# DeepLearnPhysics/u-resnet

Measured on AMD Instinct MI355X. Metric: fwd+bwd images/sec on 3D 192^3x1 U-ResNet, higher is better.
Workload: dtype f32

## Files before the change

### u-resnet_amd/csrc/conv_api.hip

```cpp
#include <dlfcn.h>
#include <stdarg.h>
#include <stdlib.h>
#include <stdio.h>
#include <string.h>

#include "bf16_common.h"

static thread_local char g_err[1024] = "";
void ursn_set_error(const char* fmt, ...) {
  va_list ap;
  va_start(ap, fmt);
  vsnprintf(g_err, sizeof(g_err), fmt, ap);
  va_end(ap);
}
extern "C" const char* ursn_last_error(void) { return g_err; }
static thread_local const char* g_kernel = "";
static long g_kernel_launches = 0;
void ursn_note_kernel(const char* name) { g_kernel = name; ++g_kernel_launches; }
void ursn_relabel_kernel(const char* name) { g_kernel = name; }
long ursn_kernel_launch_count() { return g_kernel_launches; }
extern "C" const char* ursn_last_kernel_name() { return g_kernel; }
extern "C" int ursn_abi_version(void) { return URSN_ABI_VERSION; }

namespace {
// ... 192 lines not shown
              ++nt;
            }
        g.ntaps = nt;
      }
  return ncls;
}

int conv_dispatch(const ursn_conv_desc& d, ConvPass pass, const float* in, const float* w, float* out, int accumulate,
                  hipStream_t s);

static int run_gather(const ursn_conv_desc& d, ConvPass pass, const float* in, const float* w, float* out,
                      int accumulate, hipStream_t s) {
  GatherGeom g[8];
  int n = build_geoms(d, pass, g);
  if (n < 0) return 2;
  for (int i = 0; i < n; ++i) {
    g[i].accumulate = accumulate;
    if (g[i].ntaps == 0 && accumulate) continue;
    if (d.algo == 1) URSN_TRY(launch_gconv_naive(g[i], in, w, out, s));
    else URSN_TRY(launch_gconv_mfma(g[i], in, w, out, s));
  }
  return 0;
}

int tiled_conv_supported(const ursn_conv_desc& d, ConvPass pass);
int launch_tiled_conv(const ursn_conv_desc& d, ConvPass pass, const float* in, const float* w, float* out,
                      int accumulate, hipStream_t s);

static float* op_scratch_floats(size_t n) {
  static float* buf = nullptr;
  static size_t cap = 0;
  if (n > cap) {
    if (buf) (void)hipFree(buf);
    buf = nullptr; cap = 0;
    if (hipMalloc((void**)&buf, n * sizeof(float)) != hipSuccess) return nullptr;
    cap = n;
  }
  return buf;
}

int conv_dispatch(const ursn_conv_desc& d, ConvPass pass, const float* in, const float* w, float* out, int accumulate,
                  hipStream_t s) {
  if (d.vdz_z) {
    URSN_REQUIRE(pass == PASS_DGRAD && d.vdz_coef && d.vdz_out && tiled_conv_supported(d, pass), "conv: BatchNorm-backward apply on load (vdz_z) not supported for this shape / pass");
    return launch_tiled_conv(d, pass, in, w, out, accumulate, s);
  }
  if (d.bs_partial) {
    URSN_REQUIRE(pass == PASS_DGRAD && tiled_conv_supported(d, pass), "conv: fused BatchNorm-backward reductions (bs_partial) not supported for this shape / pass");
    return launch_tiled_conv(d, pass, in, w, out, accumulate, s);
  }
  if (d.in_mean && pass != PASS_DGRAD) {
    URSN_REQUIRE(d.in_rstd && d.in_beta && tiled_conv_supported(d, pass), "conv: normalise-on-load (in_mean) not supported for this shape / pass");
    return launch_tiled_conv(d, pass, in, w, out, accumulate, s);
  }
  if (d.pw_dy) {
    URSN_REQUIRE(pass == PASS_DGRAD, "conv: fused pointwise term (pw_dy) applies to the data gradient only");
    if (tiled_deconv_supported(d, pass))
      return launch_tiled_deconv(d, pass, in, w, out, accumulate, nullptr, 0.f, nullptr, nullptr, s);
    if (!d.in_split && igemm_conv_supported(d, pass))
      return launch_igemm_conv(d, pass, in, w, out, accumulate, nullptr, 0.f, nullptr, nullptr, s);
    URSN_REQUIRE(tiled_conv_supported(d, pass), "conv: fused pointwise term (pw_dy) not supported for this shape");
    return launch_tiled_conv(d, pass, in, w, out, accumulate, s);
  }
  if (d.in_split) {
    if (pointwise_conv_supported(d, pass, accumulate))
      return launch_pointwise_conv(d, pass, in, w, out, accumulate, nullptr, 0.f, nullptr, nullptr, s);
    URSN_REQUIRE(tiled_conv_supported(d, pass), "conv: split input (in_split=%d) not supported for this shape", d.in_split);
    return launch_tiled_conv(d, pass, in, w, out, accumulate, s);
  }
  if (d.algo == 3) {
    if (tiled_deconv_supported(d, pass))
      return launch_tiled_deconv(d, pass, in, w, out, accumulate, nullptr, 0.f, nullptr, nullptr, s);
    URSN_REQUIRE(tiled_conv_supported(d, pass), "tiled conv kernel does not support this shape");
    return launch_tiled_conv(d, pass, in, w, out, accumulate, s);
  }
  if (d.algo == 4) {
    URSN_REQUIRE(igemm_conv_supported(d, pass), "igemm conv kernel does not support this shape");
    return launch_igemm_conv(d, pass, in, w, out, accumulate, nullptr, 0.f, nullptr, nullptr, s);
  }
  if (d.algo == 7) {
    URSN_REQUIRE(lds_scatter_supported(d, pass), "LDS scatter conv kernel does not support this shape");
    return launch_lds_scatter(d, pass, in, w, out, accumulate, nullptr, 0.f, nullptr, nullptr, s);
  }
  if (d.algo == 6) {
    URSN_REQUIRE(stride2_conv_supported(d, pass), "stride-2 conv kernel does not support this shape");
    return launch_stride2_conv(d, pass, in, w, out, accumulate, nullptr, 0.f, nullptr, nullptr, s);
  }
  if ((d.algo == 0 || d.algo == 5) && pointwise_conv_supported(d, pass, accumulate))
    return launch_pointwise_conv(d, pass, in, w, out, accumulate, nullptr, 0.f, nullptr, nullptr, s);
  URSN_REQUIRE(d.algo != 5, "pointwise conv kernel does not support this shape");
  if (d.algo == 0 && deep_conv_supported(d, pass)) {
    float* sc = op_scratch_floats(deep_conv_scratch_floats(d, pass));
    URSN_REQUIRE(sc, "conv: no memory for the deep-level kernel's packed weights");
    return launch_deep_conv(d, pass, in, w, out, accumulate, sc, nullptr, 0.f, nullptr, nullptr, s);
  }
  if (d.algo == 0 && igemm_conv_supported(d, pass))
    return launch_igemm_conv(d, pass, in, w, out, accumulate, nullptr, 0.f, nullptr, nullptr, s);
  if (d.algo == 0 && tiled_conv_supported(d, pass)) return launch_tiled_conv(d, pass, in, w, out, accumulate, s);
  if (d.algo == 0 && prefer_lds_scatter(d, pass))
    return launch_lds_scatter(d, pass, in, w, out, accumulate, nullptr, 0.f, nullptr, nullptr, s);
  if (d.algo == 0 && tiled_deconv_supported(d, pass))
    return launch_tiled_deconv(d, pass, in, w, out, accumulate, nullptr, 0.f, nullptr, nullptr, s);
  if (d.algo == 0 && stride2_conv_supported(d, pass))
    return launch_stride2_conv(d, pass, in, w, out, accumulate, nullptr, 0.f, nullptr, nullptr, s);
  return run_gather(d, pass, in, w, out, accumulate, s);
}

static bf16_t* op_wpack(size_t elems) {
  static bf16_t* buf = nullptr;
  static size_t cap = 0;
  if (elems > cap) {
    if (buf) (void)hipFree(buf);
    buf = nullptr; cap = 0;
    if (hipMalloc((void**)&buf, elems * sizeof(bf16_t)) != hipSuccess) return nullptr;
    cap = elems;
  }
  return buf;
}
static void stored_weight_strides(GatherGeom& g, int Kr, int Nr) { g.w_tap_stride = Kr * Nr; g.w_sk = Nr; g.w_sn = 1; }

static int bf16_conv_op(const ursn_conv_desc& d0, ConvPass pass, const void* in, const float* w, void* out, int accumulate,
                        double* stats_partial, size_t stats_bytes, float eps, float* mean, float* rstd, hipStream_t s) {
  ursn_conv_desc d = d0;
  const bool scalar_in = d.cin == 1;
  if (scalar_in) {
    URSN_REQUIRE(pass == PASS_FWD && !d.transposed && d.k == 3 && d.stride == 1 && !d.in_mean && !d.in_split,
                 "bf16 conv: the scalar fp32 input form (cin = 1) is the k3 s1 forward pass / weight gradient only");
    d.cin = 8; d.in_cstride = 8;
  }
  if (d.in_split) {
    URSN_REQUIRE(pass == PASS_DGRAD && d.in_split == 8 && d.cin == 16 && d.dx2 && d.pw_dy,
                 "bf16 conv: a split tensor is supported as the two-tensor output (dx, dx2) of the 16 -> 8 data gradient with the fused shortcut term");
    if (d.in_cstride <= 0) d.in_cstride = 8;
  }
  GatherGeom g[8];
  const int n = build_geoms(d, pass, g);
  URSN_REQUIRE(n >= 1, "bf16 conv: bad descriptor");
  int64_t V = (int64_t)d.n;
  for (int j = 0; j < 3; ++j) V *= g[0].out_d[j];
  URSN_REQUIRE(!stats_partial || n == 1 || pass == PASS_FWD, "bf16 conv: statistics only on forward passes");
  if (d.pw_dy && n == 1 && !b3conv_ok(g[0]) && bcbconv_pw_ok(g[0])) {
    URSN_REQUIRE(pass == PASS_DGRAD && d.pw_w && !d.in_split && !d.in_mean && !stats_partial, "bf16 conv: the fused shortcut term belongs to a plain data gradient");
    bf16_t* wp = op_wpack(bcbconv_pack_elems(g[0]));
    URSN_REQUIRE(wp, "bf16 conv: no memory for the packed weights");
    g[0].accumulate = accumulate;
    return launch_bcbconv(g[0], (const bf16_t*)in, w, 0, 0, wp, (bf16_t*)out, nullptr, s, (const bf16_t*)d.pw_dy,
                          d.pw_dy_cstride > 0 ? d.pw_dy_cstride : d.cout, d.pw_w);
  }
  if (scalar_in || d.in_mean || d.pw_dy) {
    URSN_REQUIRE(n == 1 && b3conv_ok(g[0]), "bf16 conv: fused forms (cin = 1 / in_mean / pw_dy) need a 3-D k3 s1 layer with 8 / 16 channels");
    bf16_t* wp = op_wpack(b3conv_pack_elems());
    URSN_REQUIRE(wp, "bf16 conv: no memory for the packed weights");
    g[0].accumulate = accumulate;
    const int blocks = bconv_grid_blocks(g[0]);
    URSN_REQUIRE(!stats_partial || bconv_stats_scratch_doubles(g[0]) * sizeof(double) <= stats_bytes, "bf16 conv: statistics scratch too small");
    if (scalar_in && (stored_weight_strides(g[0], 1, d.cout), b0conv_ok(g[0])) && !accumulate) {
      bf16_t* wp0 = op_wpack(b0conv_pack_elems());
      URSN_REQUIRE(wp0, "bf16 conv: no memory for the packed weights");
      const int blocks0 = b0conv_grid_blocks(g[0]);
      URSN_REQUIRE(!stats_partial || (size_t)blocks0 * 32 * sizeof(double) <= stats_bytes, "bf16 conv: statistics scratch too small");
      URSN_TRY(launch_b0conv(g[0], (const float*)in, w, d.cout, wp0, (bf16_t*)out, stats_partial, s));
      if (stats_partial) URSN_TRY(launch_bn_stats_final(stats_partial, blocks0, g[0].Nn, 16, V, eps, mean, rstd, s));
      return 0;
    }
    if (scalar_in) {
      URSN_REQUIRE(g[0].K == 8, "bf16 conv: the scalar input form needs the 8-channel kernel view");
      stored_weight_strides(g[0], 1, d.cout);
// ... 18 lines not shown
  bool empty = false;
  for (int i = 0; i < n; ++i) empty = empty || g[i].ntaps == 0;
  if (empty && !accumulate) {
    URSN_REQUIRE(g[0].out_cs == g[0].Nn, "bf16 conv: overwrite with empty parity classes needs a compact output tensor");
    int64_t e = (int64_t)d.n * g[0].Nn;
    for (int j = 0; j < 3; ++j) e *= g[0].out_d[j];
    URSN_HIP(hipMemsetAsync(out, 0, (size_t)e * sizeof(bf16_t), s));
  }
  if (!stats_partial && bdeconv_ok(g, n)) {
    bf16_t* wp = op_wpack(bdeconv_pack_elems());
    URSN_REQUIRE(wp, "bf16 conv: no memory for the packed weights");
    return launch_bdeconv(g, n, (const bf16_t*)in, w, 0, 0, wp, (bf16_t*)out, nullptr, accumulate, s);
  }
  if (n == 1 && bs2k8_ok(g[0])) {
    bf16_t* wp = op_wpack(bs2k8_pack_elems());
    URSN_REQUIRE(wp, "bf16 conv: no memory for the packed weights");
    const int blocks = bs2k8_grid_blocks(g[0]);
    URSN_REQUIRE(!stats_partial || (size_t)blocks * 32 * sizeof(double) <= stats_bytes, "bf16 conv: statistics scratch too small");
    URSN_TRY(launch_bs2k8(g[0], (const bf16_t*)in, w, 0, 0, wp, (bf16_t*)out, stats_partial, accumulate, nullptr, nullptr, 0, s));
    if (stats_partial) URSN_TRY(launch_bn_stats_final(stats_partial, blocks, g[0].Nn, 16, V, eps, mean, rstd, s));
    return 0;
  }
  if (bsconv_ok(g, n)) {
    bf16_t* wp = op_wpack(bsconv_pack_elems(g, n));
    URSN_REQUIRE(wp, "bf16 conv: no memory for the packed weights");
    URSN_REQUIRE(!stats_partial || bsconv_stats_scratch_doubles(g, n) * sizeof(double) <= stats_bytes, "bf16 conv: statistics scratch too small");
    URSN_TRY(launch_bsconv(g, n, (const bf16_t*)in, w, 0, 0, wp, (bf16_t*)out, stats_partial, accumulate, s));
    if (stats_partial) URSN_TRY(bsconv_stats_finalize(g, n, stats_partial, V, eps, mean, rstd, s));
    return 0;
  }
  for (int i = 0; i < n; ++i) {
    g[i].accumulate = accumulate;
    if (g[i].ntaps == 0) continue;
    bf16_t* wp = op_wpack(bconv_pack_elems(g[i]));
    URSN_REQUIRE(wp, "bf16 conv: unsupported geometry or no memory for the packed weights");
    URSN_REQUIRE(!stats_partial || bconv_stats_scratch_doubles(g[i]) * sizeof(double) * n <= stats_bytes, "bf16 conv: statistics scratch too small");
    URSN_TRY(launch_bconv(g[i], (const bf16_t*)in, w, 0, 0, wp, (bf16_t*)out, (stats_partial && n == 1) ? stats_partial : nullptr, 0, 0, s));
    if (stats_partial && n == 1) URSN_TRY(bconv_stats_finalize(g[i], stats_partial, bconv_grid_blocks(g[i]), V, eps, mean, rstd, s));
  }
  return 0;
}

extern "C" int ursn_conv_forward(const ursn_conv_desc* d, const float* x, const float* w, float* y, void* stream) {
  URSN_REQUIRE(d && x && w && y, "conv_forward: null argument");
  if (d->dtype == 1) return bf16_conv_op(*d, PASS_FWD, x, w, y, 0, nullptr, 0, 0.f, nullptr, nullptr, (hipStream_t)stream);
  return conv_dispatch(*d, PASS_FWD, x, w, y, 0, (hipStream_t)stream);
}

extern "C" int ursn_conv_forward_stats(const ursn_conv_desc* d, const float* x, const float* w, float* y, float* mean,
                                       float* rstd, float eps, void* scratch, size_t scratch_bytes, void* stream) {
  URSN_REQUIRE(d && x && w && y && mean && rstd && scratch, "conv_forward_stats: null argument");
  hipStream_t s = (hipStream_t)stream;
  if (d->dtype == 1) {
    URSN_REQUIRE(!d->transposed, "conv_forward_stats: bf16 transposed convs take their statistics at net level");
    return bf16_conv_op(*d, PASS_FWD, x, w, y, 0, (double*)scratch, scratch_bytes, eps, mean, rstd, s);
  }
  GatherGeom g[8];
  URSN_REQUIRE(build_geoms(*d, PASS_FWD, g) >= 1, "conv_forward_stats: bad descriptor");
  int64_t V = (int64_t)d->n;
  for (int j = 0; j < 3; ++j) V *= g[0].out_d[j];
  if (d->transposed) { V = (int64_t)d->n; for (int j = 0; j < d->ndim; ++j) V *= 2 * d->in_sp[j]; }
  const int ocs = d->out_cstride > 0 ? d->out_cstride : d->cout;
  if (d->in_mean)
    URSN_REQUIRE(d->in_rstd && d->in_beta && tiled_conv_supported(*d, PASS_FWD), "conv_forward_stats: normalise-on-load (in_mean) not supported for this shape");
  if (d->in_split)
    URSN_REQUIRE(pointwise_conv_supported(*d, PASS_FWD, 0) || tiled_conv_supported(*d, PASS_FWD),
                 "conv_forward_stats: split input (in_split=%d) not supported for this shape", d->in_split);
  if ((d->algo == 0 || d->algo == 5 || d->in_split) && pointwise_conv_supported(*d, PASS_FWD, 0)) {
    URSN_REQUIRE(pointwise_stats_scratch_doubles(*d) * sizeof(double) <= scratch_bytes,
                 "conv_forward_stats: scratch too small");
    return launch_pointwise_conv(*d, PASS_FWD, x, w, y, 0, (double*)scratch, eps, mean, rstd, s);
  }
  if (d->algo == 0 && deep_conv_supported(*d, PASS_FWD)) {
    URSN_REQUIRE(deep_conv_stats_scratch_doubles(*d) * sizeof(double) <= scratch_bytes, "conv_forward_stats: scratch too small");
    float* sc = op_scratch_floats(deep_conv_scratch_floats(*d, PASS_FWD));
    URSN_REQUIRE(sc, "conv_forward_stats: no memory for the deep-level kernel's packed weights");
    return launch_deep_conv(*d, PASS_FWD, x, w, y, 0, sc, (double*)scratch, eps, mean, rstd, s);
  }
  if ((d->algo == 0 || d->algo == 4) && igemm_conv_supported(*d, PASS_FWD)) {
    URSN_REQUIRE(igemm_stats_scratch_doubles(*d) * sizeof(double) <= scratch_bytes,
                 "conv_forward_stats: scratch too small");
    return launch_igemm_conv(*d, PASS_FWD, x, w, y, 0, (double*)scratch, eps, mean, rstd, s);
  }
  if ((d->algo == 0 || d->algo == 6) && stride2_conv_supported(*d, PASS_FWD)) {
    URSN_REQUIRE(stride2_stats_scratch_doubles(*d) * sizeof(double) <= scratch_bytes,
                 "conv_forward_stats: scratch too small");
    return launch_stride2_conv(*d, PASS_FWD, x, w, y, 0, (double*)scratch, eps, mean, rstd, s);
  }
  if ((d->algo == 0 && prefer_lds_scatter(*d, PASS_FWD)) || (d->algo == 7 && lds_scatter_supported(*d, PASS_FWD))) {
    URSN_REQUIRE(lds_scatter_stats_scratch_doubles(*d) * sizeof(double) <= scratch_bytes,
                 "conv_forward_stats: scratch too small");
    return launch_lds_scatter(*d, PASS_FWD, x, w, y, 0, (double*)scratch, eps, mean, rstd, s);
  }
  if ((d->algo == 0 || d->algo == 3) && tiled_deconv_supported(*d, PASS_FWD)) {
    URSN_REQUIRE(tiled_deconv_stats_scratch_doubles(*d) * sizeof(double) <= scratch_bytes,
                 "conv_forward_stats: scratch too small");
    return launch_tiled_deconv(*d, PASS_FWD, x, w, y, 0, (double*)scratch, eps, mean, rstd, s);
  }
  if ((d->algo == 0 || d->algo == 3 || d->in_split || d->in_mean) && tiled_conv_supported(*d, PASS_FWD)) {
    URSN_REQUIRE(tiled_conv_stats_scratch_doubles(*d) * sizeof(double) <= scratch_bytes,
                 "conv_forward_stats: scratch too small");
    return launch_tiled_conv_bn(*d, x, w, y, (double*)scratch, eps, mean, rstd, s);
  }
  URSN_REQUIRE(reduce_scratch_bytes(V, d->cout, 2) <= scratch_bytes, "conv_forward_stats: scratch too small");
  URSN_TRY(conv_dispatch(*d, PASS_FWD, x, w, y, 0, s));
  return launch_bn_stats(y, ocs, V, d->cout, eps, mean, rstd, scratch, s);
}

extern "C" int ursn_conv_backward_data(const ursn_conv_desc* d, const float* dy, const float* w, float* dx,
                                       int32_t accumulate, void* stream) {
  URSN_REQUIRE(d && dy && w && dx, "conv_backward_data: null argument");
  if (d->dtype == 1) return bf16_conv_op(*d, PASS_DGRAD, dy, w, dx, accumulate, nullptr, 0, 0.f, nullptr, nullptr, (hipStream_t)stream);
  return conv_dispatch(*d, PASS_DGRAD, dy, w, dx, accumulate, (hipStream_t)stream);
}

int tiled_wgrad_supported(const ursn_conv_desc& d);
size_t tiled_wgrad_scratch_bytes(const ursn_conv_desc& d);
int valu_wgrad_supported(const ursn_conv_desc& d);
size_t valu_wgrad_scratch_bytes(const ursn_conv_desc& d);
int launch_valu_wgrad(const ursn_conv_desc& d, const float* x, const float* dy, float* dw, void* scratch, size_t scratch_bytes,
                      hipStream_t s);
int launch_tiled_wgrad(const ursn_conv_desc& d, const float* x, const float* dy, float* dw, void* scratch,
                       size_t scratch_bytes, hipStream_t s);

extern "C" int32_t ursn_conv_bs_blocks(const ursn_conv_desc* d) { return d ? tiled_conv_bs_blocks(*d) : 0; }

extern "C" int ursn_conv_plan(const ursn_conv_desc* d0, int32_t pass_, char* out, size_t cap) {
  URSN_REQUIRE(d0 && out && cap > 0 && pass_ >= 0 && pass_ <= 2, "conv_plan: bad argument");
  const ConvPass pass = (ConvPass)pass_;
  ursn_conv_desc d = *d0;
  const char* name = "gather";
  GatherGeom g[8];
  if (d.dtype == 1) {
    if (d.cin == 1) { d.cin = 8; d.in_cstride = 8; }
    const int n = build_geoms(d, pass, g);
    URSN_REQUIRE(n >= 1, "conv_plan: bad descriptor");
    int first = 0;
    while (first < n - 1 && g[first].ntaps == 0) ++first;
    if (pass == PASS_WGRAD) name = (d0->cin == 1 && b0wgrad_ok(g[0])) ? "b0wgrad" : b3wgrad_ok(g[0]) ? "b3wgrad" : bdwgrad_ok(g[0]) ? "bdwgrad" : bs2k8w_ok(g[0]) ? "bs2k8w" : (bwgrad_scratch_bytes(g[0]) ? "bwgrad" : "none");
    else if (d0->cin == 1 && pass == PASS_FWD && n == 1 && b0conv_ok(g[0])) name = "b0conv";
    else if (n == 1 && bs2k8_ok(g[0])) name = "bs2k8";
    else if (bdeconv_ok(g, n)) name = "bdeconv";
    else if (bsconv_ok(g, n)) name = "bsconv";
    else if (bpw_ok(g[first])) name = "bpw";
    else if (b3conv_ok(g[first])) name = "b3conv";
    else if (bcbconv_ok(g[first])) name = "bcbconv";
    else if (bdconv_ok(g[first])) name = "bdconv";
    else name = bconv_pack_elems(g[first]) ? "bconv" : "none";
    snprintf(out, cap, "%s", name);
    return 0;
  }
  URSN_REQUIRE(build_geoms(d, pass, g) >= 1, "conv_plan: bad descriptor");
  if (pass == PASS_WGRAD) {
    if (d.in_mean || (d.in_split && !pointwise_wgrad_supported(d))) name = tiled_wgrad_supported(d) ? "twgrad" : "none";
    else if (pointwise_wgrad_supported(d)) name = "pwgrad";
    else if (deep_wgrad_supported(d)) name = "dwgrad";
    else if (igemm_wgrad_supported(d)) name = "igemm_wgrad";
    else if (valu_wgrad_supported(d)) name = "vwgrad";
    else if (tiled_wgrad_supported(d)) name = "twgrad";
    else if (stride2_wgrad_supported(d)) name = "s2wgrad";
    else name = "wgrad_mfma";
  } else {
    if (d.vdz_z || d.bs_partial || (d.in_mean && pass != PASS_DGRAD)) name = tiled_conv_supported(d, pass) ? "tconv" : "none";
    else if (d.pw_dy && tiled_deconv_supported(d, pass)) name = "tdeconv+pw";
    else if (d.pw_dy) name = (!d.in_split && igemm_conv_supported(d, pass)) ? "igemm" : (tiled_conv_supported(d, pass) ? "tconv" : "none");
    else if (d.in_split) name = pointwise_conv_supported(d, pass, 0) ? "pconv" : (tiled_conv_supported(d, pass) ? "tconv" : "none");
    else if (pointwise_conv_supported(d, pass, 0)) name = "pconv";
// ... 219 lines not shown
```

### u-resnet_amd/csrc/conv_stride2.hip

```cpp
#include <stdlib.h>
#include <utility>

#include "ursn_common.h"

typedef float s2_f32x4 __attribute__((ext_vector_type(4)));

template <int MODE> struct SBox;
template <> struct SBox<3> { static constexpr int BZ = 2, BY = 4, BX = 16, NT = 27, KZ = 3; };
template <> struct SBox<2> { static constexpr int BZ = 1, BY = 16, BX = 16, NT = 9, KZ = 1; };

struct S2Geom {
  int N, IZ, IY, IX, OZ, OY, OX, pz, py, px;
  int nbz, nby, nbx;
};

struct S2Args {
  const float* in;
  const float* w;
  float* out;
  double* stats_partial;
  S2Geom g;
  int cin, cout;
  int in_cs, out_cs;
  int accumulate;
  int nboxes, bpw;
};

template <int N, class F, int... I>
__device__ __forceinline__ void s2_static_for_impl(F&& f, std::integer_sequence<int, I...>) {
  (f(std::integral_constant<int, I>{}), ...);
}
template <int N, class F>
__device__ __forceinline__ void s2_static_for(F&& f) {
  s2_static_for_impl<N>(f, std::make_integer_sequence<int, N>{});
}

template <int MODE, int NTHR = 256>
struct HaloGeom {
  using B = SBox<MODE>;
  static constexpr int HZ = (B::KZ == 3) ? 2 * B::BZ + 1 : 1, HY = 2 * B::BY + 1, HX = 2 * B::BX + 1, HXH = B::BX + 1;
  static constexpr int PS = HZ * HY * 2 * HXH;
  static constexpr int NLD = HZ * HY * HX * 2;
  static constexpr int NH = (NLD + NTHR - 1) / NTHR;
};

struct BoxPos { int n, z0, y0, x0; };
__device__ __forceinline__ BoxPos s2_box(const S2Geom& g, int box, int BZ, int BY, int BX) {
  BoxPos b;
  const int bx = box % g.nbx; box /= g.nbx;
  const int by = box % g.nby; box /= g.nby;
  const int bz = box % g.nbz;
  b.n = box / g.nbz;
  b.x0 = bx * BX; b.y0 = by * BY; b.z0 = bz * BZ;
  return b;
}

template <int MODE, int NTHR = 256>
__device__ __forceinline__ void s2_load_halo(const float* __restrict__ src, int cs, int c0, const S2Geom& g, const BoxPos& bp,
                                             const int (&goff)[HaloGeom<MODE, NTHR>::NH], int tid,
                                             s2_f32x4 (&hv)[HaloGeom<MODE, NTHR>::NH]) {
  using H = HaloGeom<MODE, NTHR>;
  constexpr int KZ = SBox<MODE>::KZ;
  const int oz0 = (KZ == 3) ? 2 * bp.z0 - g.pz : 0, oy0 = 2 * bp.y0 - g.py, ox0 = 2 * bp.x0 - g.px;
  const int64_t base = ((((int64_t)bp.n * g.IZ + oz0) * g.IY + oy0) * g.IX + ox0) * cs + c0;
  const bool interior = oz0 >= 0 && oz0 + H::HZ <= g.IZ && oy0 >= 0 && oy0 + H::HY <= g.IY && ox0 >= 0 && ox0 + H::HX <= g.IX;
  if (interior) {
#pragma unroll
    for (int i = 0; i < H::NH; ++i) {
      s2_f32x4 v = {0.f, 0.f, 0.f, 0.f};
      if ((i + 1) * NTHR <= H::NLD || tid + i * NTHR < H::NLD) v = *(const s2_f32x4*)(src + base + goff[i]);
      hv[i] = v;
    }
  } else {
#pragma unroll
    for (int i = 0; i < H::NH; ++i) {
      const int idx = tid + i * NTHR;
      const int sv = idx >> 1;
      const int hx = sv % H::HX, r = sv / H::HX;
      const int hy = r % H::HY, hz = r / H::HY;
      const int pz = oz0 + hz, py = oy0 + hy, px = ox0 + hx;
      s2_f32x4 v = {0.f, 0.f, 0.f, 0.f};
      if (idx < H::NLD && pz >= 0 && pz < g.IZ && py >= 0 && py < g.IY && px >= 0 && px < g.IX)
        v = *(const s2_f32x4*)(src + base + goff[i]);
      hv[i] = v;
    }
  }
// ... 263 lines not shown
  s2_f32x4 hv[NH], wv[NWL];
  BoxPos cur = s2_box(g, box_begin, BZ, BY, BX);
  load_halo(cur, 0, hv);
  load_w(0, wv);
  int box = box_begin, ch = 0;
  for (int it = 0; it < nitems; ++it) {
    if (it) __syncthreads();
    store_halo(hv);
    if (it == 0 || nchunks > 1) store_w(wv);
    __syncthreads();
    int nbox = box, nch = ch + 1;
    if (nch == nchunks) { nch = 0; ++nbox; }
    BoxPos nxt = cur;
    if (it + 1 < nitems) {
      if (nbox != box) nxt = s2_box(g, nbox, BZ, BY, BX);
      load_halo(nxt, CC * nch, hv);
      if (nchunks > 1) load_w(CC * nch, wv);
    }
    if (ch == 0) {
#pragma unroll
      for (int v = 0; v < NR; ++v) acc[v] = (s2_f32x4){0.f, 0.f, 0.f, 0.f};
    }
    s2_static_for<NG>([&](auto Gi) {
      constexpr int gi = decltype(Gi)::value;
      constexpr int t0 = C16 ? gi : 2 * gi, t1 = C16 ? gi : (2 * gi + 1 < NT ? 2 * gi + 1 : NT - 1);
      constexpr int tz0 = (KZ == 3) ? t0 / 9 : 0, ty0 = (t0 / 3) % 3, tx0 = t0 % 3;
      constexpr int tz1 = (KZ == 3) ? t1 / 9 : 0, ty1 = (t1 / 3) % 3, tx1 = t1 % 3;
      constexpr int toff0 = ((tz0 * HY + ty0) * 2 + (tx0 & 1)) * HXH + (tx0 >> 1);
      constexpr int toff1 = ((tz1 * HY + ty1) * 2 + (tx1 & 1)) * HXH + (tx1 >> 1);
      const int toff = second ? toff1 : toff0;
      s2_f32x4 av = wl[wb + (second ? t1 : t0) * (NPC * WST)];
      if (!C16 && 2 * gi + 1 >= NT && second) av = (s2_f32x4){0.f, 0.f, 0.f, 0.f};
#pragma unroll
      for (int v = 0; v < NR; ++v) {
        const s2_f32x4 bv = hal[hb[v] + toff];
#pragma unroll
        for (int j = 0; j < 4; ++j) acc[v] = __builtin_amdgcn_mfma_f32_16x16x4f32(av[j], bv[j], acc[v], 0, 0, 0);
      }
    });
    if (ch == nchunks - 1) {
      const int gx = cur.x0 + il;
#pragma unroll
      for (int v = 0; v < NR; ++v) {
        const int row = NR * wave + v;
        const int gz = (MODE == 3) ? cur.z0 + row / BY : 0, gy = (MODE == 3) ? cur.y0 + row % BY : cur.y0 + row;
        if (!(gz < g.OZ && gy < g.OY && gx < g.OX)) continue;
        float* op = a.out + ((((size_t)cur.n * g.OZ + gz) * g.OY + gy) * g.OX + gx) * a.out_cs + co0 + 4 * kl;
        s2_f32x4 val = acc[v];
        if (a.accumulate) val += *(s2_f32x4*)op;
        *(s2_f32x4*)op = val;
        if constexpr (STATS) {
#pragma unroll
          for (int r = 0; r < 4; ++r) {
            if (nacc == 0.f) piv[r] = val[r];
            ursn_sacc(piv[r], s1[r], s2[r], val[r]);
          }
          nacc += 1.f;
        }
      }
    }
    box = nbox; ch = nch; cur = nxt;
  }
  if constexpr (STATS) {
    __shared__ double red[NWAVE][32];
#pragma unroll
    for (int r = 0; r < 4; ++r) {
      double u, w2;
      ursn_sacc_final(piv[r], s1[r], s2[r], nacc, u, w2);
#pragma unroll
      for (int o = 8; o >= 1; o >>= 1) { u += __shfl_xor(u, o); w2 += __shfl_xor(w2, o); }
      if (il == 0) {
        red[wave][4 * kl + r] = u;
        red[wave][16 + 4 * kl + r] = w2;
      }
    }
    __syncthreads();
    if (tid < 32)
      a.stats_partial[((size_t)blockIdx.y * gridDim.x + blockIdx.x) * 32 + tid] =
          ((red[0][tid] + red[1][tid]) + (red[2][tid] + red[3][tid])) +
          ((red[4][tid] + red[5][tid]) + (red[6][tid] + red[7][tid]));
  }
}

struct S2WArgs {
  const float* S;
  const float* C;
  float* slab;
  S2Geom g;
  int s_cs, c_cs;
  int nboxes, bpg;
};

template <int MODE>
__global__ __launch_bounds__(256, 2) void s2wgrad_kernel(S2WArgs a) {
  using B = SBox<MODE>;
  using H = HaloGeom<MODE>;
  constexpr int BZ = B::BZ, BY = B::BY, BX = B::BX, NT = B::NT, KZ = B::KZ;
  constexpr int HY = H::HY, HX = H::HX, HXH = H::HXH, PS = H::PS, NLD = H::NLD, NH = H::NH;
  constexpr int DS = BZ * BY * BX, NLC = DS * 4, NC = (NLC + 255) / 256;
  constexpr int NP = (NT + 1) / 2;
  constexpr int NQW = DS / 16;
  extern __shared__ __attribute__((aligned(16))) float s2w[];
  float* sl = s2w;
  float* cl = s2w + PS * 8;

  const int tid = threadIdx.x, lane = tid & 63, wave = tid >> 6;
  const int il = lane & 15, kl = lane >> 4;
  const S2Geom& g = a.g;
  const int ci0 = blockIdx.y * 8, co0 = blockIdx.z * 16;

  int goff[NH], loff[NH];
#pragma unroll
  for (int i = 0; i < NH; ++i) {
    const int idx = tid + i * 256;
    const int sv = idx >> 1, q = idx & 1;
    const int hx = sv % HX, r = sv / HX;
    const int hy = r % HY, hz = r / HY;
    goff[i] = ((hz * g.IY + hy) * g.IX + hx) * a.s_cs + 4 * q;
    loff[i] = (((hz * HY + hy) * 2 + (hx & 1)) * HXH + (hx >> 1)) * 8 + 4 * q;
  }
  int coff[NC];
#pragma unroll
  for (int i = 0; i < NC; ++i) {
    const int idx = tid + i * 256;
    const int vox = idx >> 2, q = idx & 3;
    const int vx = vox % BX, r = vox / BX;
    const int vy = r % BY, vz = r / BY;
    coff[i] = ((vz * g.OY + vy) * g.OX + vx) * a.c_cs + 4 * q;
  }

  const int row0 = (NQW / 4) * wave;
  const int lz0 = (MODE == 3) ? row0 / BY : 0, ly0 = (MODE == 3) ? row0 % BY : row0;
  s2_f32x4 acc[NP];
  int t_off[NP];
#pragma unroll
  for (int m = 0; m < NP; ++m) {
    acc[m] = (s2_f32x4){0.f, 0.f, 0.f, 0.f};
    int t = 2 * m + (il >> 3);
    if (t >= NT) t = NT - 1;
    const int tz = (KZ == 3) ? t / 9 : 0, ty = (t / 3) % 3, tx = t % 3;
    t_off[m] = ((((2 * lz0 + tz) * HY + 2 * ly0 + ty) * 2 + (tx & 1)) * HXH + (tx >> 1) + kl) * 8 + (il & 7);
  }
  const int b_off = ((row0 * BX) + kl) * 16 + il;

  auto load_box = [&](const BoxPos& bp, s2_f32x4 (&sv4)[NH], s2_f32x4 (&cv4)[NC]) {
    s2_load_halo<MODE>(a.S, a.s_cs, ci0, g, bp, goff, tid, sv4);
    const int64_t cbase = ((((int64_t)bp.n * g.OZ + bp.z0) * g.OY + bp.y0) * g.OX + bp.x0) * a.c_cs + co0;
    const bool interior = bp.z0 + BZ <= g.OZ && bp.y0 + BY <= g.OY && bp.x0 + BX <= g.OX;
#pragma unroll
    for (int i = 0; i < NC; ++i) {
      const int idx = tid + i * 256;
      bool ok = (i + 1) * 256 <= NLC || idx < NLC;
      if (!interior) {
        const int vox = idx >> 2;
        const int vx = vox % BX, r = vox / BX;
        const int vy = r % BY, vz = r / BY;
        ok = ok && bp.z0 + vz < g.OZ && bp.y0 + vy < g.OY && bp.x0 + vx < g.OX;
      }
      s2_f32x4 v = {0.f, 0.f, 0.f, 0.f};
      if (ok) v = *(const s2_f32x4*)(a.C + cbase + coff[i]);
      cv4[i] = v;
    }
  };
  auto store_box = [&](const s2_f32x4 (&sv4)[NH], const s2_f32x4 (&cv4)[NC]) {
#pragma unroll
    for (int i = 0; i < NH; ++i)
// ... 10 lines not shown
  if (box_end > a.nboxes) box_end = a.nboxes;
  s2_f32x4 sv4[NH], cv4[NC];
  if (box_begin < box_end) load_box(s2_box(g, box_begin, BZ, BY, BX), sv4, cv4);
  for (int box = box_begin; box < box_end; ++box) {
    __syncthreads();
    store_box(sv4, cv4);
    __syncthreads();
    if (box + 1 < box_end) load_box(s2_box(g, box + 1, BZ, BY, BX), sv4, cv4);
    s2_static_for<NQW>([&](auto J) {
      constexpr int j = decltype(J)::value;
      constexpr int dr = j >> 2, xq = (j & 3) * 4;
      const float bv = cl[b_off + (dr * BX + xq) * 16];
#pragma unroll
      for (int m = 0; m < NP; ++m) {
        const float av = sl[t_off[m] + ((2 * dr) * 2 * HXH + xq) * 8];
        acc[m] = __builtin_amdgcn_mfma_f32_16x16x4f32(av, bv, acc[m], 0, 0, 0);
      }
    });
  }

  __syncthreads();
  float* red = s2w;
  for (int i = tid; i < NT * 128; i += 256) red[i] = 0.f;
  __syncthreads();
  for (int w = 0; w < 4; ++w) {
    if (wave == w) {
#pragma unroll
      for (int m = 0; m < NP; ++m)
#pragma unroll
        for (int r = 0; r < 4; ++r) {
          const int row = 4 * kl + r, t = 2 * m + (row >> 3);
          if (t < NT) red[(t * 8 + (row & 7)) * 16 + il] += acc[m][r];
        }
    }
    __syncthreads();
  }
  float* slab = a.slab + (((size_t)blockIdx.z * gridDim.y + blockIdx.y) * gridDim.x + blockIdx.x) * (size_t)(NT * 128);
  for (int i = tid; i < NT * 128; i += 256) slab[i] = red[i];
}

__global__ __launch_bounds__(256) void s2w_reduce_kernel(float* __restrict__ dw, const float* __restrict__ slab, int taps,
                                                         int K, int Nn, int ng) {
  __shared__ float sm[4][64];
  const int e = threadIdx.x & 63, cg = threadIdx.x >> 6;
  const int64_t total = (int64_t)taps * K * Nn;
  const int64_t i = (int64_t)blockIdx.x * 64 + e;
  float s0 = 0.f, s1 = 0.f;
  if (i < total) {
    const int co = (int)(i % Nn);
    const int64_t r = i / Nn;
    const int ci = (int)(r % K);
    const int t = (int)(r / K);
    const int cy = ci / 8, cz = co / 16, ncy = K / 8;
    const int64_t per = (int64_t)taps * 128;
    const float* base = slab + ((int64_t)(cz * ncy + cy) * ng) * per + ((int64_t)t * 8 + (ci & 7)) * 16 + (co & 15);
    int gi = cg;
    for (; gi + 4 < ng; gi += 8) {
      s0 += base[(int64_t)gi * per];
      s1 += base[(int64_t)(gi + 4) * per];
    }
    for (; gi < ng; gi += 4) s0 += base[(int64_t)gi * per];
  }
  sm[cg][e] = s0 + s1;
  __syncthreads();
  if (cg == 0 && i < total) dw[i] += (sm[0][e] + sm[1][e]) + (sm[2][e] + sm[3][e]);
}

struct S2Plan {
  int mode, K, Nn, in_cs, out_cs;
  S2Geom g;
  int nboxes, bpw, gridx;
  size_t lds_conv, lds_wgrad;
  int ngroups, bpg;
  size_t scratch;
};

static bool s2_enabled(const ursn_conv_desc& d) {
  static int off = -1;
  if (off < 0) {
    const char* e = getenv("URSN_DISABLE_TILED");
    const char* f = getenv("URSN_STRIDE2");
    off = ((e && e[0] == '1') || (f && f[0] == '0')) ? 1 : 0;
  }
  return !off || d.algo == 6;
}

static bool make_s2plan(const ursn_conv_desc& d, S2Plan& p) {
  if (!s2_enabled(d)) return false;
  if (d.k != 3 || d.stride != 2 || d.in_split || d.in_mean) return false;
  if (d.ndim != 2 && d.ndim != 3) return false;
  const int ics = d.in_cstride > 0 ? d.in_cstride : d.cin, ocs = d.out_cstride > 0 ? d.out_cstride : d.cout;
  p.mode = d.ndim;
  p.K = d.transposed ? d.cout : d.cin;
  p.Nn = d.transposed ? d.cin : d.cout;
  p.in_cs = d.transposed ? ocs : ics;
  p.out_cs = d.transposed ? ics : ocs;
  if ((p.K % 8) || (p.Nn % 16) || (p.in_cs & 3) || (p.out_cs & 3)) return false;
  int hi[3] = {1, 1, 1}, lo[3] = {1, 1, 1}, pb[3] = {0, 0, 0};
  const int lead = 3 - d.ndim;
  for (int j = 0; j < d.ndim; ++j) {
    const int sz = d.in_sp[j];
    if (sz < 1) return false;
    if (d.transposed) { lo[lead + j] = sz; hi[lead + j] = 2 * sz; pb[lead + j] = 0; }
    else {
      const int o = (sz + 1) / 2;
      int tot = (o - 1) * 2 + 3 - sz;
      if (tot < 0) tot = 0;
      hi[lead + j] = sz; lo[lead + j] = o; pb[lead + j] = tot / 2;
    }
  }
  S2Geom& g = p.g;
  g.N = d.n;
  g.IZ = hi[0]; g.IY = hi[1]; g.IX = hi[2];
  g.OZ = lo[0]; g.OY = lo[1]; g.OX = lo[2];
  g.pz = pb[0]; g.py = pb[1]; g.px = pb[2];
  static const int minx = getenv("URSN_S2_MINX") ? atoi(getenv("URSN_S2_MINX")) : 8;
  if (g.OX < minx && d.algo != 6) return false;
  const int BZ = p.mode == 3 ? 2 : 1, BY = p.mode == 3 ? 4 : 16, BX = 16;
  g.nbz = (g.OZ + BZ - 1) / BZ;
  g.nby = (g.OY + BY - 1) / BY;
  g.nbx = (g.OX + BX - 1) / BX;
  const int64_t nb = (int64_t)d.n * g.nbz * g.nby * g.nbx;
  if (nb > (1 << 30)) return false;
  p.nboxes = (int)nb;
  const int NT = p.mode == 3 ? 27 : 9;
  const int HZ = p.mode == 3 ? 2 * BZ + 1 : 1, HY = 2 * BY + 1, HXH = BX + 1;
  const int PS = HZ * HY * 2 * HXH;
  const int PSP = PS + ((16 - PS % 32) + 32) % 32;
  p.lds_conv = ((size_t)8 * PSP + (size_t)NT * 128) * sizeof(float);
  p.bpw = (int)(((int64_t)p.nboxes * (p.Nn / 16)) / 2048);
  if (p.bpw < 1) p.bpw = 1;
  if (p.bpw > 8) p.bpw = 8;
  p.gridx = (p.nboxes + p.bpw - 1) / p.bpw;
  p.lds_wgrad = ((size_t)PS * 8 + (size_t)BZ * BY * BX * 16) * sizeof(float);
  const int blocks = (p.K / 8) * (p.Nn / 16);
  int want = 1024 / blocks;
  if (want < 1) want = 1;
  if (want > p.nboxes) want = p.nboxes;
  p.bpg = (p.nboxes + want - 1) / want;
  p.ngroups = (p.nboxes + p.bpg - 1) / p.bpg;
  p.scratch = (size_t)blocks * p.ngroups * NT * 128 * sizeof(float);
  return p.scratch <= ((size_t)1 << 30);
}

int stride2_conv_supported(const ursn_conv_desc& d, ConvPass pass) {
  if (!((!d.transposed && pass == PASS_FWD) || (d.transposed && pass == PASS_DGRAD))) return 0;
  S2Plan p;
  return make_s2plan(d, p) ? 1 : 0;
}

size_t stride2_stats_scratch_doubles(const ursn_conv_desc& d) {
  S2Plan p;
  if (d.transposed || !make_s2plan(d, p)) return 0;
  return (size_t)p.gridx * (p.Nn / 16) * 32;
}

template <int MODE, bool STATS>
static int launch_s2c(const S2Plan& p, const S2Args& a, hipStream_t s) {
  auto kern = s2conv_kernel<MODE, STATS>;
  static size_t attr_lds = 48 * 1024;
  if (p.lds_conv > attr_lds) {
    URSN_HIP(hipFuncSetAttribute((const void*)kern, hipFuncAttributeMaxDynamicSharedMemorySize, (int)p.lds_conv));
    attr_lds = p.lds_conv;
  }
  hipLaunchKernelGGL(kern, dim3(p.gridx, p.Nn / 16), dim3(512), p.lds_conv, s, a);
  URSN_HIP(hipGetLastError());
  return 0;
}

template <int MODE, bool C16, bool STATS>
static int launch_s2c2(const S2Plan& p, const S2Args& a, hipStream_t s) {
  using H = Halo2<MODE, C16, 512>;
  constexpr int NT = SBox<MODE>::NT;
  const size_t lds = ((size_t)H::NPC * H::PSP + (size_t)NT * H::NPC * H::WST) * 16;
  auto kern = s2conv2_kernel<MODE, C16, STATS>;
  static size_t attr_lds = 48 * 1024;
  if (lds > attr_lds) {
    URSN_HIP(hipFuncSetAttribute((const void*)kern, hipFuncAttributeMaxDynamicSharedMemorySize, (int)lds));
    attr_lds = lds;
  }
  hipLaunchKernelGGL(kern, dim3(p.gridx, p.Nn / 16), dim3(512), lds, s, a);
  URSN_HIP(hipGetLastError());
  return 0;
}

int launch_stride2_conv(const ursn_conv_desc& d, ConvPass pass, const float* in, const float* w, float* out,
                        int accumulate, double* stats_partial, float eps, float* mean, float* rstd, hipStream_t s) {
  S2Plan p;
  URSN_REQUIRE(stride2_conv_supported(d, pass) && make_s2plan(d, p), "stride-2 conv: unsupported shape");
  S2Args a;
  a.in = in; a.w = w; a.out = out; a.stats_partial = stats_partial;
  a.g = p.g;
  a.cin = p.K; a.cout = p.Nn; a.in_cs = p.in_cs; a.out_cs = p.out_cs;
  a.accumulate = accumulate;
  a.nboxes = p.nboxes; a.bpw = p.bpw;
  ursn_note_kernel(d.transposed ? "s2conv(deconv dgrad)" : "s2conv");
  int rc;
  static const int v2mode = getenv("URSN_S2CONV_V2") ? atoi(getenv("URSN_S2CONV_V2")) : 1;
  const bool v2 = v2mode == 2 || (v2mode == 1 && p.mode == 2 && (p.K == 32 || p.K == 64));
  if (v2) {
    const bool c16 = (p.K % 16) == 0;
#define S2V2(m_, c_) (stats_partial ? launch_s2c2<m_, c_, true>(p, a, s) : launch_s2c2<m_, c_, false>(p, a, s))
    if (p.mode == 3) rc = c16 ? S2V2(3, true) : S2V2(3, false);
    else rc = c16 ? S2V2(2, true) : S2V2(2, false);
#undef S2V2
  } else if (p.mode == 3) rc = stats_partial ? launch_s2c<3, true>(p, a, s) : launch_s2c<3, false>(p, a, s);
  else rc = stats_partial ? launch_s2c<2, true>(p, a, s) : launch_s2c<2, false>(p, a, s);
  if (rc) return rc;
  if (stats_partial) {
    const int64_t V = (int64_t)d.n * p.g.OZ * p.g.OY * p.g.OX;
    URSN_TRY(launch_bn_stats_final_blocked(stats_partial, p.gridx, p.Nn, 16, 16, (size_t)p.gridx * 32, V, eps, mean, rstd, s));
  }
  return 0;
}

int stride2_wgrad_supported(const ursn_conv_desc& d) {
  S2Plan p;
  return make_s2plan(d, p) ? 1 : 0;
}
size_t stride2_wgrad_scratch_bytes(const ursn_conv_desc& d) {
  S2Plan p;
  return make_s2plan(d, p) ? p.scratch : 0;
}

template <int MODE>
static int launch_s2w(const S2Plan& p, const S2WArgs& a, dim3 grid, hipStream_t s) {
  auto kern = s2wgrad_kernel<MODE>;
  static size_t attr_lds = 48 * 1024;
  if (p.lds_wgrad > attr_lds) {
    URSN_HIP(hipFuncSetAttribute((const void*)kern, hipFuncAttributeMaxDynamicSharedMemorySize, (int)p.lds_wgrad));
    attr_lds = p.lds_wgrad;
  }
  hipLaunchKernelGGL(kern, grid, dim3(256), p.lds_wgrad, s, a);
  URSN_HIP(hipGetLastError());
  return 0;
}

int launch_stride2_wgrad(const ursn_conv_desc& d, const float* x, const float* dy, float* dw, void* scratch,
                         size_t scratch_bytes, hipStream_t s) {
  S2Plan p;
  URSN_REQUIRE(make_s2plan(d, p), "stride-2 wgrad: unsupported shape");
  URSN_REQUIRE(scratch && scratch_bytes >= p.scratch, "stride-2 wgrad: scratch too small (%zu < %zu)", scratch_bytes, p.scratch);
  S2WArgs a;
  a.S = d.transposed ? dy : x;
  a.C = d.transposed ? x : dy;
  a.slab = (float*)scratch;
  a.g = p.g;
  a.s_cs = p.in_cs; a.c_cs = p.out_cs;
  a.nboxes = p.nboxes; a.bpg = p.bpg;
  dim3 grid(p.ngroups, p.K / 8, p.Nn / 16);
  ursn_note_kernel("s2wgrad");
  URSN_TRY(p.mode == 3 ? launch_s2w<3>(p, a, grid, s) : launch_s2w<2>(p, a, grid, s));
  const int taps = p.mode == 3 ? 27 : 9;
  const int64_t total = (int64_t)taps * p.K * p.Nn;
  hipLaunchKernelGGL(s2w_reduce_kernel, dim3((unsigned)cdiv64(total, 64)), dim3(256), 0, s, dw, (const float*)scratch, taps,
                     p.K, p.Nn, p.ngroups);
  URSN_HIP(hipGetLastError());
  return 0;
}
```

Measured before the change: 68.03.

## Add z-streaming stride-2 conv kernel with rolling halo planes and separate stats pass

Adds a new stride-2 3x3x3 conv kernel for small input-channel counts (K=8 or 16). Each block walks a chunk of output z-slices and keeps three rotating LDS halo planes, so each input z-plane is loaded once and reused across neighbouring outputs. The next plane pair is prefetched through buffer loads while the current slice's MFMAs run. Weights for the block's output channels stay resident in LDS. Batch-norm statistics move to a separate pass that rereads the output, which adds memory traffic when stats are needed. The path is used by default (algo 0) for transposed dgrad with K=8 and for K=16 mode-3 shapes, and is also selectable with algo 8.

Result: no change. 68.10 (median of 6 runs) (+0.1%).

```diff
diff --git a/u-resnet_amd/csrc/conv_api.hip b/u-resnet_amd/csrc/conv_api.hip
--- a/u-resnet_amd/csrc/conv_api.hip
+++ b/u-resnet_amd/csrc/conv_api.hip
@@ -298,7 +298,7 @@
     URSN_REQUIRE(lds_scatter_supported(d, pass), "LDS scatter conv kernel does not support this shape");
     return launch_lds_scatter(d, pass, in, w, out, accumulate, nullptr, 0.f, nullptr, nullptr, s);
   }
-  if (d.algo == 6) {
+  if (d.algo == 6 || d.algo == 8) {
     URSN_REQUIRE(stride2_conv_supported(d, pass), "stride-2 conv kernel does not support this shape");
     return launch_stride2_conv(d, pass, in, w, out, accumulate, nullptr, 0.f, nullptr, nullptr, s);
   }
@@ -483,7 +483,7 @@
                  "conv_forward_stats: scratch too small");
     return launch_igemm_conv(*d, PASS_FWD, x, w, y, 0, (double*)scratch, eps, mean, rstd, s);
   }
-  if ((d->algo == 0 || d->algo == 6) && stride2_conv_supported(*d, PASS_FWD)) {
+  if ((d->algo == 0 || d->algo == 6 || d->algo == 8) && stride2_conv_supported(*d, PASS_FWD)) {
     URSN_REQUIRE(stride2_stats_scratch_doubles(*d) * sizeof(double) <= scratch_bytes,
                  "conv_forward_stats: scratch too small");
     return launch_stride2_conv(*d, PASS_FWD, x, w, y, 0, (double*)scratch, eps, mean, rstd, s);
diff --git a/u-resnet_amd/csrc/conv_stride2.hip b/u-resnet_amd/csrc/conv_stride2.hip
--- a/u-resnet_amd/csrc/conv_stride2.hip
+++ b/u-resnet_amd/csrc/conv_stride2.hip
@@ -2,6 +2,7 @@
 #include <utility>
 
 #include "ursn_common.h"
+#include "buffer_stage.h"
 
 typedef float s2_f32x4 __attribute__((ext_vector_type(4)));
 
@@ -431,6 +432,194 @@
   }
 }
 
+#define URSN_S2Z_OOB_YX 0x40000000u
+#define URSN_S2Z_OOB_Z 0x80000000u
+template <int K, int TY>
+struct ZGeom {
+  static constexpr int NCO = 8 / TY;
+  static constexpr int HY = 2 * TY + 1, HX = 33, HXH = 17;
+  static constexpr int PS = HY * 2 * HXH;
+  static constexpr int PSP = PS + ((16 - PS % 32) + 32) % 32;
+  static constexpr int SL = K * PSP;
+  static constexpr int NLD = 2 * HY * HX * (K / 4);
+  static constexpr int NH = (NLD + 511) / 512;
+  static constexpr int NW4 = 27 * NCO * K * 4;
+  static constexpr size_t LDS = ((size_t)3 * SL + (size_t)NW4 * 4) * sizeof(float);
+};
+
+struct S2ZArgs {
+  const float* in;
+  const float* w;
+  float* out;
+  S2Geom g;
+  int cout, in_cs, out_cs, zc;
+};
+
+template <int K, int TY, bool ACC>
+__global__ __launch_bounds__(512, (K <= 8 ? 2 : 1)) void s2zconv_kernel(S2ZArgs a) {
+  using Z = ZGeom<K, TY>;
+  constexpr int NCO = Z::NCO, HY = Z::HY, HX = Z::HX, HXH = Z::HXH, PSP = Z::PSP, SL = Z::SL, NLD = Z::NLD, NH = Z::NH;
+  extern __shared__ __attribute__((aligned(16))) float s2l[];
+  float* hal = s2l;
+  float* wl = s2l + 3 * SL;
+
+  const int tid = threadIdx.x, lane = tid & 63, wave = tid >> 6;
+  const int il = lane & 15, kl = lane >> 4;
+  const int row = wave % TY, ct = wave / TY;
+  const S2Geom& g = a.g;
+  const int co0 = blockIdx.y * (16 * NCO);
+
+  int b = ursn_xcd_block(blockIdx.x, gridDim.x);
+  const int bx = b % g.nbx; b /= g.nbx;
+  const int by = b % g.nby; b /= g.nby;
+  const int bz = b % g.nbz;
+  const int n = b / g.nbz;
+  const int x0 = bx * 16, y0 = by * TY, oz0 = bz * a.zc;
+  int oz1 = oz0 + a.zc;
+  if (oz1 > g.OZ) oz1 = g.OZ;
+  const int ox0 = 2 * x0 - g.px, oy0 = 2 * y0 - g.py, hz0 = 2 * oz0 - g.pz;
+
+  for (int i = tid; i < Z::NW4; i += 512) {
+    const int c4 = i & 3, k = (i >> 2) % K, tc = (i >> 2) / K;
+    const int c = tc % NCO, t = tc / NCO;
+    *(s2_f32x4*)(wl + 4 * i) = *(const s2_f32x4*)(a.w + ((size_t)t * K + k) * a.cout + co0 + 16 * c + 4 * c4);
+  }
+
+  const unsigned plane = (unsigned)g.IY * g.IX * a.in_cs * 4u;
+  unsigned boff[NH];
+  int loff[NH];
+  unsigned ppm = 0;
+#pragma unroll
+  for (int i = 0; i < NH; ++i) {
+    const int idx = tid + i * 512;
+    const int q = idx % (K / 4), sv = idx / (K / 4);
+    const int hx = sv % HX, r = sv / HX;
+    const int hy = r % HY, pp = r / HY;
+    const int py = oy0 + hy, px = ox0 + hx;
+    const bool ok = idx < NLD && py >= 0 && py < g.IY && px >= 0 && px < g.IX;
+    boff[i] = ok ? (unsigned)((py * g.IX + px) * a.in_cs + 4 * q) * 4u : URSN_S2Z_OOB_YX;
+    loff[i] = 4 * q * PSP + (hy * 2 + (hx & 1)) * HXH + (hx >> 1);
+    if (pp) ppm |= 1u << i;
+  }
+  const __amdgpu_buffer_rsrc_t rsrc = ursn_plane_rsrc(a.in + (size_t)n * g.IZ * g.IY * g.IX * a.in_cs, (unsigned)g.IZ * plane);
+
+  s2_f32x4 hv[NH];
+  auto load_pair = [&](int h, bool one) {
+    const int z0 = hz0 + h;
+    const unsigned zo0 = (z0 >= 0 && z0 < g.IZ) ? (unsigned)z0 * plane : URSN_S2Z_OOB_Z;
+    const unsigned zo1 = (!one && z0 + 1 >= 0 && z0 + 1 < g.IZ) ? (unsigned)(z0 + 1) * plane : URSN_S2Z_OOB_Z;
+#pragma unroll
+    for (int i = 0; i < NH; ++i) hv[i] = ursn_buffer_load_f4(rsrc, (((ppm >> i) & 1) ? zo1 : zo0) + boff[i]);
+  };
+  auto store_pair = [&](int sa, int sb, bool one) {
+#pragma unroll
+    for (int i = 0; i < NH; ++i) {
+      if (((i + 1) * 512 <= NLD || tid + i * 512 < NLD) && !(one && ((ppm >> i) & 1))) {
+        float* d = hal + (((ppm >> i) & 1) ? sb : sa) + loff[i];
+#pragma unroll
+        for (int j = 0; j < 4; ++j) d[j * PSP] = hv[i][j];
+      }
+    }
+  };
+  const int nst = oz1 - oz0;
+  load_pair(0, false);
+  store_pair(0, SL, false);
+  load_pair(2, true);
+  store_pair(2 * SL, 0, true);
+  __syncthreads();
+
+  const int hb = kl * PSP + (2 * row) * 2 * HXH + il;
+  const int wb = (ct * K + kl) * 16 + il;
+  const int gy = y0 + row, gx = x0 + il;
+  const bool st_ok = gy < g.OY && gx < g.OX;
+  float* op = a.out + ((((size_t)n * g.OZ + oz0) * g.OY + gy) * g.OX + gx) * a.out_cs + co0 + 16 * ct + 4 * kl;
+  const size_t ostep = (size_t)g.OY * g.OX * a.out_cs;
+  auto emit = [&](const s2_f32x4& acc, const s2_f32x4& old) {
+    if (st_ok) *(s2_f32x4*)op = acc + old;
+    op += ostep;
+  };
+  auto prior = [&]() {
+    s2_f32x4 v = {0.f, 0.f, 0.f, 0.f};
+    if (ACC && st_ok) v = *(const s2_f32x4*)op;
+    return v;
+  };
+  s2_f32x4 acc = {0.f, 0.f, 0.f, 0.f};
+  int s0 = 0;
+#pragma unroll 1
+  for (int r = 0; r < nst; ++r) {
+    const bool more = r + 1 < nst;
+    const s2_f32x4 old = r ? prior() : acc;
+    if (more) load_pair(2 * r + 3, false);
+    if (r) emit(acc, old);
+    const int sa = s0 * SL, sb = (s0 == 2 ? 0 : s0 + 1) * SL, sc = (s0 == 0 ? 2 : s0 - 1) * SL;
+    acc = (s2_f32x4){0.f, 0.f, 0.f, 0.f};
+#pragma unroll
+    for (int c8 = 0; c8 < K; c8 += 8) {
+      s2_static_for<27>([&](auto T) {
+        constexpr int t = decltype(T)::value;
+        constexpr int tz = t / 9, ty = (t / 3) % 3, tx = t % 3;
+        constexpr int toff = (ty * 2 + (tx & 1)) * HXH + (tx >> 1);
+        const int sbase = tz == 0 ? sa : (tz == 1 ? sb : sc);
+#pragma unroll
+        for (int s = 0; s < 2; ++s) {
+          const float av = wl[wb + ((t * NCO) * K + c8 + 4 * s) * 16];
+          const float bv = hal[sbase + hb + (c8 + 4 * s) * PSP + toff];
+          acc = __builtin_amdgcn_mfma_f32_16x16x4f32(av, bv, acc, 0, 0, 0);
+        }
+      });
+    }
+    if (more) {
+      __syncthreads();
+      store_pair(sa, sb, false);
+      __syncthreads();
+    }
+    s0 = s0 == 0 ? 2 : s0 - 1;
+  }
+  if (nst > 0) emit(acc, prior());
+}
+
+__global__ __launch_bounds__(512) void s2zstats_kernel(S2Args a) {
+  constexpr int NWAVE = 8, BZ = 2, BY = 4, BX = 16;
+  const int tid = threadIdx.x, lane = tid & 63, wave = tid >> 6;
+  const int il = lane & 15, kl = lane >> 4;
+  const S2Geom& g = a.g;
+  const int co0 = blockIdx.y * 16;
+  const int box_begin = ursn_xcd_block(blockIdx.x, gridDim.x) * a.bpw;
+  int box_end = box_begin + a.bpw;
+  if (box_end > a.nboxes) box_end = a.nboxes;
+  float s1[4] = {0.f, 0.f, 0.f, 0.f}, s2[4] = {0.f, 0.f, 0.f, 0.f}, piv[4] = {0.f, 0.f, 0.f, 0.f}, nacc = 0.f;
+  for (int box = box_begin; box < box_end; ++box) {
+    const BoxPos cur = s2_box(g, box, BZ, BY, BX);
+    const int gx = cur.x0 + il, gz = cur.z0 + wave / BY, gy = cur.y0 + wave % BY;
+    if (!(gz < g.OZ && gy < g.OY && gx < g.OX)) continue;
+    const s2_f32x4 val =
+        *(const s2_f32x4*)(a.out + ((((size_t)cur.n * g.OZ + gz) * g.OY + gy) * g.OX + gx) * a.out_cs + co0 + 4 * kl);
+#pragma unroll
+    for (int r = 0; r < 4; ++r) {
+      if (nacc == 0.f) piv[r] = val[r];
+      ursn_sacc(piv[r], s1[r], s2[r], val[r]);
+    }
+    nacc += 1.f;
+  }
+  __shared__ double red[NWAVE][32];
+#pragma unroll
+  for (int r = 0; r < 4; ++r) {
+    double u, w2;
+    ursn_sacc_final(piv[r], s1[r], s2[r], nacc, u, w2);
+#pragma unroll
+    for (int o = 8; o >= 1; o >>= 1) { u += __shfl_xor(u, o); w2 += __shfl_xor(w2, o); }
+    if (il == 0) {
+      red[wave][4 * kl + r] = u;
+      red[wave][16 + 4 * kl + r] = w2;
+    }
+  }
+  __syncthreads();
+  if (tid < 32)
+    a.stats_partial[((size_t)blockIdx.y * gridDim.x + blockIdx.x) * 32 + tid] =
+        ((red[0][tid] + red[1][tid]) + (red[2][tid] + red[3][tid])) +
+        ((red[4][tid] + red[5][tid]) + (red[6][tid] + red[7][tid]));
+}
+
 struct S2WArgs {
   const float* S;
   const float* C;
@@ -607,7 +796,7 @@
     const char* f = getenv("URSN_STRIDE2");
     off = ((e && e[0] == '1') || (f && f[0] == '0')) ? 1 : 0;
   }
-  return !off || d.algo == 6;
+  return !off || d.algo == 6 || d.algo == 8;
 }
 
 static bool make_s2plan(const ursn_conv_desc& d, S2Plan& p) {
@@ -640,7 +829,7 @@
   g.OZ = lo[0]; g.OY = lo[1]; g.OX = lo[2];
   g.pz = pb[0]; g.py = pb[1]; g.px = pb[2];
   static const int minx = getenv("URSN_S2_MINX") ? atoi(getenv("URSN_S2_MINX")) : 8;
-  if (g.OX < minx && d.algo != 6) return false;
+  if (g.OX < minx && d.algo != 6 && d.algo != 8) return false;
   const int BZ = p.mode == 3 ? 2 : 1, BY = p.mode == 3 ? 4 : 16, BX = 16;
   g.nbz = (g.OZ + BZ - 1) / BZ;
   g.nby = (g.OY + BY - 1) / BY;
@@ -668,10 +857,44 @@
   return p.scratch <= ((size_t)1 << 30);
 }
 
+struct S2ZPlan {
+  S2Geom g;
+  int ty, zc, gridx, gridy;
+};
+
+static bool make_s2zplan(const ursn_conv_desc& d, const S2Plan& p, S2ZPlan& z) {
+  if (d.algo != 0 && d.algo != 8) return false;
+  if (p.mode != 3 || !((p.K == 8 && p.Nn % 16 == 0) || (p.K == 16 && p.Nn % 32 == 0))) return false;
+  if (d.algo == 0 && !d.transposed && p.K == 8) return false;
+  if ((int64_t)p.g.IZ * p.g.IY * p.g.IX * p.in_cs * 4 >= ((int64_t)1 << 30)) return false;
+  z.g = p.g;
+  z.ty = p.K == 8 ? 8 : 4;
+  z.g.nby = (p.g.OY + z.ty - 1) / z.ty;
+  z.g.nbx = (p.g.OX + 15) / 16;
+  z.gridy = p.Nn / (p.K == 8 ? 16 : 32);
+  const int64_t tiles = (int64_t)p.g.N * z.g.nby * z.g.nbx * z.gridy;
+  const int64_t slots = 256 * (p.K == 8 ? 2 : 1);
+  double best = 0.0;
+  z.zc = p.g.OZ;
+  for (int zc = 1; zc <= p.g.OZ; ++zc) {
+    const int64_t nbz = (p.g.OZ + zc - 1) / zc;
+    const int64_t rounds = (tiles * nbz + slots - 1) / slots;
+    const double cost = (double)rounds * (2 * zc + 3);
+    if (zc == 1 || cost < best) { best = cost; z.zc = zc; }
+  }
+  z.g.nbz = (p.g.OZ + z.zc - 1) / z.zc;
+  const int64_t gx = tiles / z.gridy * z.g.nbz;
+  if (gx > (1 << 30)) return false;
+  z.gridx = (int)gx;
+  return true;
+}
+
 int stride2_conv_supported(const ursn_conv_desc& d, ConvPass pass) {
   if (!((!d.transposed && pass == PASS_FWD) || (d.transposed && pass == PASS_DGRAD))) return 0;
   S2Plan p;
-  return make_s2plan(d, p) ? 1 : 0;
+  if (!make_s2plan(d, p)) return 0;
+  S2ZPlan z;
+  return (d.algo != 8 || make_s2zplan(d, p, z)) ? 1 : 0;
 }
 
 size_t stride2_stats_scratch_doubles(const ursn_conv_desc& d) {
@@ -709,10 +932,52 @@
   return 0;
 }
 
+template <int K, int TY, bool ACC>
+static int launch_s2z(const S2ZPlan& z, const S2ZArgs& a, hipStream_t s) {
+  constexpr size_t lds = ZGeom<K, TY>::LDS;
+  auto kern = s2zconv_kernel<K, TY, ACC>;
+  static bool attr = false;
+  if (!attr) {
+    URSN_HIP(hipFuncSetAttribute((const void*)kern, hipFuncAttributeMaxDynamicSharedMemorySize, (int)lds));
+    attr = true;
+  }
+  hipLaunchKernelGGL(kern, dim3(z.gridx, z.gridy), dim3(512), lds, s, a);
+  URSN_HIP(hipGetLastError());
+  return 0;
+}
+
 int launch_stride2_conv(const ursn_conv_desc& d, ConvPass pass, const float* in, const float* w, float* out,
                         int accumulate, double* stats_partial, float eps, float* mean, float* rstd, hipStream_t s) {
   S2Plan p;
   URSN_REQUIRE(stride2_conv_supported(d, pass) && make_s2plan(d, p), "stride-2 conv: unsupported shape");
+  S2ZPlan z;
+  if (make_s2zplan(d, p, z)) {
+    S2ZArgs a;
+    a.in = in; a.w = w; a.out = out;
+    a.g = z.g;
+    a.cout = p.Nn; a.in_cs = p.in_cs; a.out_cs = p.out_cs;
+    a.zc = z.zc;
+    ursn_note_kernel(d.transposed ? "s2zconv(deconv dgrad)" : "s2zconv");
+    int rc;
+    URSN_REQUIRE(!(stats_partial && accumulate), "stride-2 conv: statistics of an accumulated output");
+#define S2Z(k_, ty_) (accumulate ? launch_s2z<k_, ty_, true>(z, a, s) : launch_s2z<k_, ty_, false>(z, a, s))
+    if (p.K == 8) rc = S2Z(8, 8);
+    else rc = S2Z(16, 4);
+#undef S2Z
+    if (rc) return rc;
+    if (stats_partial) {
+      S2Args sa;
+      sa.out = out; sa.stats_partial = stats_partial;
+      sa.g = p.g;
+      sa.out_cs = p.out_cs;
+      sa.nboxes = p.nboxes; sa.bpw = p.bpw;
+      hipLaunchKernelGGL(s2zstats_kernel, dim3(p.gridx, p.Nn / 16), dim3(512), 0, s, sa);
+      URSN_HIP(hipGetLastError());
+      const int64_t V = (int64_t)d.n * p.g.OZ * p.g.OY * p.g.OX;
+      URSN_TRY(launch_bn_stats_final_blocked(stats_partial, p.gridx, p.Nn, 16, 16, (size_t)p.gridx * 32, V, eps, mean, rstd, s));
+    }
+    return 0;
+  }
   S2Args a;
   a.in = in; a.w = w; a.out = out; a.stats_partial = stats_partial;
   a.g = p.g;
```
